# arpg/Kangaroo

Hardware: AMD Instinct MI355X
Metric: kinectfusion_frames_per_sec_640x480_to_512cubed_tsdf (higher is better)
Workload: dtype f32

## Files before the change

include/kfx_debug.h:

```cpp
#ifndef KFX_DEBUG_H
#define KFX_DEBUG_H

#include "kfx.h"

#ifdef __cplusplus
extern "C" {
#endif

int kfx_debug_rmw(const kfx_volume* vol, int variant, kfx_stream stream);

int kfx_debug_div_uniform_check(float b, unsigned long long* d_out, kfx_stream stream);

int kfx_debug_div_core_check(unsigned seed, int per_divisor, unsigned long long* d_out, kfx_stream stream);
int kfx_debug_sqrt_core_check(unsigned long long* d_out, kfx_stream stream);
int kfx_debug_wave_xor_check(unsigned seed, unsigned long long* d_out, kfx_stream stream);

int kfx_debug_summary_export(kfx_sdf_summary* s, float tol, float vref, int fine_shift, void* R_out, void* C_out, int dims_out[12],
                             kfx_stream stream);

int kfx_debug_summary_conditional_builds(kfx_sdf_summary* s, int out[2], kfx_stream stream);

#ifdef __cplusplus
}
#endif
#endif
```

kangaroo_amd/csrc/debug.hip:

```cpp
#include "kfx_device.h"
#include "sampling.h"
#include "../../include/kfx_debug.h"

namespace kfx {

__global__ __launch_bounds__(256) void k_rmw_linear(float4* __restrict__ base, size_t n4)
{
    const size_t stride = (size_t)gridDim.x * blockDim.x;
    for (size_t i = (size_t)blockIdx.x * blockDim.x + threadIdx.x; i < n4; i += stride) {
        float4 c = base[i];
        c.y += 1.0f;
        c.w += 1.0f;
        base[i] = c;
    }
}

template <int ZC>
__global__ __launch_bounds__(256) void k_rmw_brick(unsigned char* vptr, size_t pitch, size_t img_pitch, int X, int Y, int Z)
{
    const int tid = threadIdx.x, lane = tid & 63, wv = tid >> 6;
    const int x0 = (blockIdx.x * 32 + (lane & 31)) * 2;
    const int y = blockIdx.y * 8 + wv * 2 + (lane >> 5);
    const int zbeg = blockIdx.z * ZC, zend = min(zbeg + ZC, Z);
    if (x0 >= X || y >= Y) return;
// ... 203 lines not shown
    }
    case 1: hipLaunchKernelGGL(k_rmw_brick<16>, dim3(ceil_div(X, 64), ceil_div(Y, 8), ceil_div(Z, 16)), dim3(256), 0, s, p, vol->pitch, vol->img_pitch, X, Y, Z); break;
    case 2: hipLaunchKernelGGL(k_rmw_rows<16>, dim3(ceil_div(X, 128), ceil_div(Y, 4), ceil_div(Z, 16)), dim3(256), 0, s, p, vol->pitch, vol->img_pitch, X, Y, Z); break;
    case 3: hipLaunchKernelGGL(k_rmw_column, dim3(ceil_div(X, 128), ceil_div(Y, 4), 1), dim3(256), 0, s, p, vol->pitch, vol->img_pitch, X, Y, Z); break;
    case 4: hipLaunchKernelGGL(k_rmw_brick<64>, dim3(ceil_div(X, 64), ceil_div(Y, 8), ceil_div(Z, 64)), dim3(256), 0, s, p, vol->pitch, vol->img_pitch, X, Y, Z); break;
    case 5: hipLaunchKernelGGL(k_rmw_rows<4>, dim3(ceil_div(X, 128), ceil_div(Y, 4), ceil_div(Z, 4)), dim3(256), 0, s, p, vol->pitch, vol->img_pitch, X, Y, Z); break;
#define GEN(ID, WX, WY, ZC, NT) \
    case ID: hipLaunchKernelGGL((k_rmw_gen<WX, WY, ZC, NT>), dim3(ceil_div(X, 128 * WX), ceil_div(Y, WY), ceil_div(Z, ZC)), dim3(256), 0, s, p, vol->pitch, vol->img_pitch, X, Y, Z); break;
    GEN(10, 4, 1, 16, false)
    GEN(11, 2, 2, 16, false)
    GEN(12, 1, 4, 16, false)
    GEN(13, 1, 4, 16, true)
    GEN(14, 4, 1, 16, true)
    GEN(15, 1, 4, 1, false)
    GEN(16, 1, 4, 64, false)
    GEN(17, 4, 1, 4, false)
    GEN(18, 2, 2, 16, true)
#undef GEN
    default: return set_error(KFX_E_RANGE, "kfx_debug_rmw: variant");
    }
    return check_launch("kfx_debug_rmw");
}

extern "C" int kfx_debug_summary_export(kfx_sdf_summary* s, float tol, float vref, int fine_shift, void* R_out, void* C_out, int dims_out[12],
                                        kfx_stream stream)
{
    if (!s || !dims_out) return set_error(KFX_E_NULL, "kfx_debug_summary_export: null argument");
    if (fine_shift < 3 || fine_shift > 5) return set_error(KFX_E_RANGE, "kfx_debug_summary_export: fine_shift in [3, 5]");
    ClassView cv;
    summary_class_layout(s, fine_shift, cv);
    dims_out[0] = s->nbx; dims_out[1] = s->nby; dims_out[2] = s->nbz;
    dims_out[3] = cv.fine.first; dims_out[4] = cv.fine.rw; dims_out[5] = cv.fine.ny;
    dims_out[6] = cv.coarse.first; dims_out[7] = cv.coarse.rw; dims_out[8] = cv.coarse.ny;
    dims_out[9] = cv.words; dims_out[10] = s->n_coarse; dims_out[11] = (s->h_skippable && s->builds) ? ((volatile int*)s->h_skippable)[(s->builds - 1) % KFX_SUMMARY_RING] : -2;
    const size_t n = (size_t)s->nbx * s->nby * s->nbz;
    hipStream_t st = (hipStream_t)stream;
    if (R_out && hipMemcpyAsync(R_out, s->R, n * sizeof(float4), hipMemcpyDeviceToDevice, st) != hipSuccess) return set_error(KFX_E_RANGE, "kfx_debug_summary_export: copy");
    if (C_out) {
        if (int e = summary_classes_prepare(s, tol, vref, fine_shift, st)) return e;
        if (hipMemcpyAsync(C_out, s->C, (size_t)cv.words * sizeof(unsigned), hipMemcpyDeviceToDevice, st) != hipSuccess || hipStreamSynchronize(st) != hipSuccess)
            return set_error(KFX_E_RANGE, "kfx_debug_summary_export: copy");
        dims_out[11] = (s->h_skippable && s->builds) ? ((volatile int*)s->h_skippable)[(s->builds - 1) % KFX_SUMMARY_RING] : -2;
    }
    return 0;
}

extern "C" int kfx_debug_summary_conditional_builds(kfx_sdf_summary* s, int out[2], kfx_stream stream)
{
    if (!s || !out) return set_error(KFX_E_NULL, "kfx_debug_summary_conditional_builds: null argument");
    hipStream_t st = (hipStream_t)stream;
    if (hipMemcpyAsync(out, s->d_count + 3, 2 * sizeof(int), hipMemcpyDeviceToHost, st) != hipSuccess || hipStreamSynchronize(st) != hipSuccess)
        return set_error(KFX_E_RANGE, "kfx_debug_summary_conditional_builds: copy");
    return 0;
}
```

kangaroo_amd/csrc/kfx_device.h:

```cpp
#pragma once

#include <hip/hip_runtime.h>
#include <stddef.h>
#include <stdint.h>

#include "../../include/kfx.h"
#include "../../include/kfx_extras.h"
#include "../../include/kfx_summary_h.h"

namespace kfx {

struct V3 { float x, y, z; };

__device__ __forceinline__ V3 v3(float x, float y, float z) { return V3{x, y, z}; }
__device__ __forceinline__ V3 operator+(V3 a, V3 b) { return V3{a.x + b.x, a.y + b.y, a.z + b.z}; }
__device__ __forceinline__ V3 operator-(V3 a, V3 b) { return V3{a.x - b.x, a.y - b.y, a.z - b.z}; }
__device__ __forceinline__ V3 operator*(V3 a, float s) { return V3{a.x * s, a.y * s, a.z * s}; }
__device__ __forceinline__ V3 div_cw(V3 a, V3 b) { return V3{a.x / b.x, a.y / b.y, a.z / b.z}; }
__device__ __forceinline__ V3 div_s(V3 a, float s) { const float inv = 1.0f / s; return a * inv; }
__device__ __forceinline__ float dot(V3 a, V3 b) { return a.x * b.x + a.y * b.y + a.z * b.z; }
__device__ __forceinline__ float length(V3 a) { return sqrtf(dot(a, a)); }
__device__ __forceinline__ float lerp(float a, float b, float t) { return a + t * (b - a); }
__device__ __forceinline__ V3 lerp(V3 a, V3 b, float t) { return a + (b - a) * t; }
__device__ __forceinline__ float clampf(float f, float a, float b) { return fmaxf(a, fminf(f, b)); }
// ... 138 lines not shown
};

__host__ __device__ inline int ceil_div(int a, int b) { return (a + b - 1) / b; }

}

#define KFX_SUMMARY_RING 8
struct kfx_sdf_summary {
    float4* R;
    int nbx, nby, nbz;
    int w, h, d;
    int cell_bytes;
    const unsigned char* base;
    size_t pitch, img_pitch;
    unsigned* C;
    int c_dirty;
    float c_lo_ok, c_hi_ok;
    float c_tol, c_vref;
    int c_shift;
    int c_global;
    int n_coarse;
    int* d_count;
    int* d_dirty;
    int* h_skippable;
    int* d_skippable;
    hipEvent_t build_done[8];
    unsigned builds;
    unsigned plain_calls;
    unsigned sweeps;
};
namespace kfx {
struct ClassLevel {
    int shift;
    int ny;
    int rw;
    int first;
};
struct ClassView {
    const unsigned* C;
    ClassLevel fine, coarse;
    int words;
    float vref;
    float tol;
    int amb_ok;
    int ox, oy, oz;
    float eps;
    int nx5, nz5, top_n, lds_words;
    int global, top_first;
};
__device__ __forceinline__ unsigned brick_class_mask(const float lo, const float hi, const int state, const float lo_ok, const float hi_ok)
{
    const bool in_band = lo >= lo_ok && hi <= hi_ok;
    return (state == 1 ? 1u : 0u) | ((state == 0 && in_band) ? 2u : 0u) | ((state == 1 || in_band) ? 4u : 0u);
}
inline __host__ __device__ void class_level_up(const int nx, const int ny, const int nz, const int shift, const int first, ClassLevel& L, int& ux, int& uz, int& words)
{
    ux = (nx + 1) >> 1; uz = (nz + 1) >> 1;
    L.shift = shift; L.ny = (ny + 1) >> 1; L.rw = 2 * ((ux + 31) >> 5); L.first = first;
    words = (L.rw * L.ny * uz + 3) & ~3;
}
__device__ __forceinline__ void classes_level_up(unsigned* tab, const ClassLevel& src, int snx, int snz, const ClassLevel& dst, int dnx, int dnz)
{
    const int lane = threadIdx.x & 63;
    int lg = 0;
    while ((1 << lg) < dnx && lg < 6) ++lg;
    const int chunks = (dnx + 63) >> 6;
    const int px = chunks > 1 ? chunks << 6 : 1 << lg;
    const int total = px * dst.ny * dnz;
    for (int e0 = 0; e0 < total; e0 += 256) {
        const int e = e0 + (int)threadIdx.x;
        const int bx = chunks > 1 ? e % px : e & (px - 1), r = chunks > 1 ? e / px : e >> lg;
        const int by = r % dst.ny, bz = r / dst.ny;
        int cls = 0;
        if (e < total && bx < dnx) {
            bool all_free = true, all_nan = true, all_either = true;
#pragma unroll
            for (int k = 0; k < 8; ++k) {
                const int x = min(2 * bx + (k & 1), snx - 1), y = min(2 * by + ((k >> 1) & 1), src.ny - 1), z = min(2 * bz + (k >> 2), snz - 1);
                const uint2 w = *reinterpret_cast<const uint2*>(tab + src.first + (z * src.ny + y) * src.rw + ((x >> 5) << 1));
                const int c = (int)((w.x >> (x & 31)) & 1u) | (int)(((w.y >> (x & 31)) & 1u) << 1);
                all_free = all_free && c == 1;
                all_nan = all_nan && c == 2;
                all_either = all_either && c != 0;
            }
            cls = all_free ? 1 : (all_nan ? 2 : (all_either ? 3 : 0));
        }
        const unsigned long long p0 = __ballot(cls & 1), p1 = __ballot(cls & 2);
        if (e < total && (bx & 63) == 0 && (chunks > 1 || bx == 0)) {
            const int sh = chunks > 1 ? 0 : lane;
            const unsigned long long m = (chunks > 1 || lg == 6) ? ~0ull : ((1ull << (1 << lg)) - 1ull);
            const unsigned long long r0 = (p0 >> sh) & m, r1 = (p1 >> sh) & m;
            unsigned* out = tab + dst.first + (bz * dst.ny + by) * dst.rw + (bx >> 6) * 4;
            out[0] = (unsigned)r0; out[1] = (unsigned)r1;
            if ((bx >> 6) * 4 + 2 < dst.rw) { out[2] = (unsigned)(r0 >> 32); out[3] = (unsigned)(r1 >> 32); }
        }
    }
}
int summary_classes_prepare(kfx_sdf_summary* s, float tol, float vref, int fine_shift, hipStream_t stream, int global = 0);
void summary_class_layout(const kfx_sdf_summary* s, int fine_shift, ClassView& cv);
void summary_top_layout(const ClassView& cv, ClassLevel& l6, ClassLevel& l7, int& w6, int& w7);
int summary_view_offset(const kfx_sdf_summary* s, const kfx_volume* view, int* ox, int* oy, int* oz);
}

namespace kfx {
int set_error(int code, const char* what);
int check_launch(const char* what);
int math_mode();
size_t texel_image_bytes(size_t w, size_t h);
int depth_to_vbo_normals_texels(const kfx_image* vbo, const kfx_image* nrm, const kfx_image* depth, const float K[4], float scale,
                                const kfx_image* texels, kfx_stream stream);
int sdf_fuse_slab_texels(const kfx_volume* vol, const kfx_slab* slab, const kfx_image* depth, const kfx_image* norm, const kfx_image* texels,
                         const float T_cw[12], const float K[4], float trunc_dist, float max_w, float mincostheta, unsigned flags, kfx_stream stream);
int sdf_fuse_texels(const kfx_volume* vol, kfx_sdf_summary* summary, const kfx_image* depth, const kfx_image* norm, const kfx_image* texels,
                    const float T_cw[12], const float K[4], float trunc_dist, float max_w, float mincostheta, unsigned flags, kfx_stream stream);
}
```

kangaroo_amd/csrc/raycast.hip:

```cpp
#include <cmath>

#include <hip/hip_fp16.h>

#include "kfx_device.h"
#include "sampling.h"

namespace kfx {

struct RayParams {
    VolView vol;
    V3 size;
    V3 dims1;
    V3 hi2;
    V3 voxel;
    V3 inv_size;
    int fastdiv, off32;
    Pose T;
    Intr K;
    unsigned char *dptr, *nptr, *iptr;
    size_t dpitch, npitch, ipitch;
    int w, h;
    float near, far, trunc;
    int subpix;
    int tile_log2w;
// ... 659 lines not shown
    if (int e = check_volume(vol, CELL::BYTES, 3, VOLUME_MAX_DIM, "RaycastSdf")) return e;
    set_geometry(p, vol);
    set_voxel_size(p, vol);
    for (int i = 0; i < 12; ++i) p.T.m[i] = T_wc[i];
    p.K = Intr{K[0], K[1], K[2], K[3]};
    p.dptr = (unsigned char*)depth->ptr;
    p.nptr = (unsigned char*)norm->ptr;
    p.iptr = (unsigned char*)img->ptr;
    p.dpitch = depth->pitch;
    p.npitch = norm->pitch;
    p.ipitch = img->pitch;
    p.w = (int)img->w;
    p.h = (int)img->h;
    p.near = near;
    p.far = far;
    p.trunc = trunc_dist;
    p.subpix = subpix ? 1 : 0;
    p.tile_log2w = 5;
    p.wg_log2x = 1;
    p.sparse_lanes = 0;
    return 0;
}

template <typename CELL>
static int class_view(ClassView& cl, size_t* lds_bytes, int* usable, kfx_sdf_summary* summary, const kfx_volume* vol, const RayParams& p, kfx_stream stream,
                      bool allow_global = true)
{
    *usable = 0;
    if (int e = summary_view_offset(summary, vol, &cl.ox, &cl.oy, &cl.oz)) return e;
    if (!(p.trunc > 0.f) || !(p.trunc < __builtin_inff())) return 0;
    static const int kb_env = env_int("KFX_RAYCAST_CLASS_KB", 16, 1, 60);
    static const int gt_env = env_int("KFX_RAYCAST_GLOBAL_TABLES", 0);
    static const int top_env = env_int("KFX_RAYCAST_TOP_LEVELS", 2, 0, 2);
    int fine = 3;
    for (; fine < 5; ++fine) {
        summary_class_layout(summary, fine, cl);
        if ((size_t)cl.words * 4 <= (size_t)kb_env * 1024) break;
    }
    auto top_levels = [&](int& w6, int& w7) {
        summary_class_layout(summary, fine, cl);
        cl.nx5 = ceil_div(summary->w, 32); cl.nz5 = ceil_div(summary->d, 32);
        ClassLevel l6, l7;
        summary_top_layout(cl, l6, l7, w6, w7);
        const int nx6 = (cl.nx5 + 1) >> 1, nz6 = (cl.nz5 + 1) >> 1;
        cl.top_n = 0;
        if (cl.nx5 > 1 || cl.coarse.ny > 1 || cl.nz5 > 1) cl.top_n = 1;
// ... 5 lines not shown
    const size_t lds_static = sizeof(RayParams) + sizeof(TopLevels) + 2048;
    const int derived = (cl.top_n > 0 ? w6 : 0) + (cl.top_n > 1 ? w7 : 0);
    cl.global = gt_env > 0 || (size_t)cl.words * 4 > 60 * 1024 || (size_t)(cl.words + derived) * 4 + lds_static > 64 * 1024;
    if (cl.global) {
        fine = 4;
        top_levels(w6, w7);
        cl.top_first = cl.words;
        cl.lds_words = (cl.top_n > 0 ? w6 : 0) + (cl.top_n > 1 ? w7 : 0);
        if ((size_t)cl.lds_words * 4 + lds_static > 64 * 1024) return 0;
    } else {
        cl.top_first = 0;
        cl.lds_words = cl.words + derived;
    }
    if (cl.global && !allow_global) return 0;
    const bool half = CELL::BYTES == 4;
    const float vref = half ? __half2float(__float2half_rn(p.trunc)) : p.trunc;
    const float tol = math_mode() == KFX_MATH_FAST ? (half ? KFX_SUMMARY_HALF_BAND : 1e-5f) : 0.f;
    static const int force_env = env_int("KFX_RAYCAST_SUMMARY", 0);
    if (force_env < 0) return 0;
    const bool steer = force_env == 0 && summary->h_skippable;
    if (steer && summary->plain_calls && (summary->plain_calls++ % 8u) != 0u) return 0;
    if (int e = summary_classes_prepare(summary, tol, vref, fine, (hipStream_t)stream, cl.global)) return e;
    if (steer && summary->builds >= 3) {
        const unsigned ref = (summary->builds - 3) % KFX_SUMMARY_RING;
        (void)hipEventSynchronize(summary->build_done[ref]);
        const int known = ((volatile int*)summary->h_skippable)[ref];
        if (known >= 0 && (long long)known * 4 < summary->n_coarse) {
            if (!summary->plain_calls) summary->plain_calls = 1;
            return 0;
        }
        summary->plain_calls = 0;
    }
    cl.C = summary->C;
    cl.vref = vref;
    cl.amb_ok = fmaxf(vref, p.voxel.x) == p.trunc ? 1 : 0;
    cl.tol = tol;
    const double u24 = 1.0 / 16777216.0;
    double eps = 0.0;
    const float bmin[3] = {p.vol.bmin.x, p.vol.bmin.y, p.vol.bmin.z}, bmax[3] = {p.vol.bmax.x, p.vol.bmax.y, p.vol.bmax.z};
    const float size[3] = {p.size.x, p.size.y, p.size.z}, dims1[3] = {p.dims1.x, p.dims1.y, p.dims1.z};
    const float cw[3] = {p.T.m[3], p.T.m[7], p.T.m[11]};
    for (int a = 0; a < 3; ++a) {
        if (!(size[a] > 0.f)) return 0;
        const double sc = (double)dims1[a] / size[a];
        const double pmax = std::fmax(std::fabs((double)bmin[a]), std::fabs((double)bmax[a])), ca = std::fabs((double)cw[a]);
        const double A = std::fabs(((double)cw[a] - bmin[a]) * sc);
        const double t = sc * (3.0 * pmax + 2.0 * ca + size[a]) * u24 + 2.0 * dims1[a] * u24;
        const double e = u24 * (3.0 * A + 2.0 * sc * (pmax + ca) + dims1[a]) + 3.0 * u24 * (dims1[a] + A);
        eps = std::fmax(eps, t + e);
// ... 347 lines not shown
```

kangaroo_amd/csrc/summary.hip:

```cpp
#include <algorithm>
#include <new>

#include <hip/hip_fp16.h>

#include "kfx_device.h"

namespace kfx {

__global__ __launch_bounds__(256) void k_summary_fill(float4* __restrict__ R, size_t n, float lo, float hi, int state)
{
    const size_t i = (size_t)blockIdx.x * 256 + threadIdx.x;
    if (i < n) R[i] = make_float4(lo, hi, __int_as_float(state), 0.f);
}

struct ClassBuild {
    const float4* R;
    unsigned* C;
    int nbx, nby, nbz;
    int shift, nx, ny, nz, rw;
    float lo_ok, hi_ok;
    const unsigned* src;
    int src_shift, src_nx, src_ny, src_nz, src_rw;
};
struct TopBuild {
    int on;
    unsigned* tab;
    ClassLevel l5, l6, l7;
    int nx5, nz5, nx6, nz6, nx7, nz7;
};
template <int M>
__device__ __forceinline__ int class_row(const ClassBuild& b, const long long wave)
{
    const float4* __restrict__ R = b.R;
    unsigned* __restrict__ C = b.C;
    const unsigned* __restrict__ src = b.src;
    const int nbx = b.nbx, nby = b.nby, nbz = b.nbz, shift = b.shift, nx = b.nx, ny = b.ny, rw = b.rw;
    const int src_shift = b.src_shift, src_nx = b.src_nx, src_ny = b.src_ny, src_nz = b.src_nz, src_rw = b.src_rw;
    const float lo_ok = b.lo_ok, hi_ok = b.hi_ok;
    const int lane = threadIdx.x & 63;
    const int chunks = (nx + 63) >> 6;
    const int chunk = (int)(wave % chunks), by = (int)((wave / chunks) % ny), bz = (int)(wave / ((long long)chunks * ny));
    const int bx = chunk * 64 + lane;
    int cls = 0;
    if (bx < nx) {
        bool all_nan = true, all_free = true, all_either = true;
        if constexpr (M == 0) {
            const int m = 1 << (shift - src_shift);
            for (int z0 = 0; z0 < m; z0 += 2) {
                uint2 w2[2][4];
#pragma unroll
                for (int dz = 0; dz < 2; ++dz)
// ... 34 lines not shown
                    for (int dx = 0; dx <= M; ++dx)
                        r[(dz * (M + 1) + dy) * (M + 1) + dx] =
                            R[((size_t)min(bz * M + dz, nbz - 1) * nby + min(by * M + dy, nby - 1)) * nbx + min(bx * M + dx, nbx - 1)];
#pragma unroll
            for (int k = 0; k < (M + 1) * (M + 1) * (M + 1); ++k) {
                const unsigned m = brick_class_mask(r[k].x, r[k].y, __float_as_int(r[k].z), lo_ok, hi_ok);
                all_nan = all_nan && (m & 1u);
                all_free = all_free && (m & 2u);
                all_either = all_either && (m & 4u);
            }
        }
        cls = all_free ? 1 : (all_nan ? 2 : (all_either ? 3 : 0));
    }
    const unsigned long long p0 = __ballot(cls & 1), p1 = __ballot(cls & 2);
    if (lane == 0) {
        unsigned* row = C + ((size_t)bz * ny + by) * rw + chunk * 4;
        row[0] = (unsigned)p0; row[1] = (unsigned)p1;
        if (chunk * 4 + 2 < rw) { row[2] = (unsigned)(p0 >> 32); row[3] = (unsigned)(p1 >> 32); }
    }
    return __popcll(p0 | p1);
}

template <int M>
__global__ __launch_bounds__(256) void k_summary_classes(const ClassBuild b, const long long n_waves, const int* __restrict__ dirty)
{
    if (dirty && *dirty == 0) return;
    const long long wave = (long long)blockIdx.x * 4 + (threadIdx.x >> 6);
    if (wave < n_waves) class_row<M>(b, wave);
}

template <int M>
__global__ __launch_bounds__(256) void k_summary_classes_coarse(const ClassBuild b, const long long n_waves, int* __restrict__ count, int* __restrict__ publish,
                                                                int* __restrict__ dirty, const int conditional, const TopBuild t)
{
    __shared__ int s_count[4];
    __shared__ int s_last;
    if (conditional && *dirty == 0) {
        if (blockIdx.x == 0 && threadIdx.x == 0) {
            __hip_atomic_store(publish, count[2], __ATOMIC_RELAXED, __HIP_MEMORY_SCOPE_SYSTEM);
            count[4] += 1;
        }
        return;
    }
    const int wv = threadIdx.x >> 6;
    const long long wave = (long long)blockIdx.x * 4 + wv;
    const int n = wave < n_waves ? class_row<M>(b, wave) : 0;
    if ((threadIdx.x & 63) == 0) s_count[wv] = n;
    __threadfence();
    __syncthreads();
    if (threadIdx.x == 0) {
        s_last = 0;
        atomicAdd(&count[0], s_count[0] + s_count[1] + s_count[2] + s_count[3]);
        __threadfence();
        if (atomicAdd(&count[1], 1) == (int)gridDim.x - 1) {
            __threadfence();
            s_last = 1;
            const int total = atomicExch(&count[0], 0);
            count[1] = 0;
            count[2] = total;
            if (conditional) count[3] += 1;
            *dirty = 0;
            __hip_atomic_store(publish, total, __ATOMIC_RELAXED, __HIP_MEMORY_SCOPE_SYSTEM);
        }
    }
    __syncthreads();
    if (t.on && s_last) {
        __threadfence();
        classes_level_up(t.tab, t.l5, t.nx5, t.nz5, t.l6, t.nx6, t.nz6);
        __threadfence();
        __syncthreads();
        classes_level_up(t.tab, t.l6, t.nx6, t.nz6, t.l7, t.nx7, t.nz7);
    }
}

template <int BYTES>
__global__ __launch_bounds__(256) void k_summary_rebuild(float4* __restrict__ R, const unsigned char* __restrict__ base, size_t pitch, size_t img_pitch,
                                                         int w, int h, int d, int nbx, int nby, int nbz, int aligned16)
{
    const long long brick = (long long)blockIdx.x * 4 + (threadIdx.x >> 6);
    if (brick >= (long long)nbx * nby * nbz) return;
    const int lane = threadIdx.x & 63;
    const int bx = (int)(brick % nbx), by = (int)((brick / nbx) % nby), bz = (int)(brick / ((long long)nbx * nby));
    const int y = by * 8 + (lane & 7), z = bz * 8 + (lane >> 3), x0 = bx * 8;
    float lo = __builtin_inff(), hi = -__builtin_inff();
    bool nan = false, val = false;
    if (y < h && z < d) {
        const unsigned char* row = base + (size_t)z * img_pitch + (size_t)y * pitch + (size_t)x0 * BYTES;
        if (BYTES == 4 && x0 + 8 <= w && aligned16) {
            uint4 c[2];
#pragma unroll
            for (int k = 0; k < 2; ++k) c[k] = reinterpret_cast<const uint4*>(row)[k];
#pragma unroll
            for (int k = 0; k < 2; ++k) {
                const unsigned u[4] = {c[k].x, c[k].y, c[k].z, c[k].w};
// ... 51 lines not shown
}
static int class_level_words(const ClassLevel& L, int d) { return L.rw * L.ny * ceil_div(d, 1 << L.shift); }

void summary_class_layout(const kfx_sdf_summary* s, int fine_shift, ClassView& cv)
{
    class_level(cv.fine, fine_shift, s->w, s->h, 0);
    const int fw = fine_shift < 5 ? class_level_words(cv.fine, s->d) : 0;
    class_level(cv.coarse, 5, s->w, s->h, (fw + 3) & ~3);
    cv.words = cv.coarse.first + ((class_level_words(cv.coarse, s->d) + 3) & ~3);
}

void summary_top_layout(const ClassView& cv, ClassLevel& l6, ClassLevel& l7, int& w6, int& w7)
{
    int nx6, nz6, nx7, nz7;
    class_level_up(cv.nx5, cv.coarse.ny, cv.nz5, 6, cv.words, l6, nx6, nz6, w6);
    class_level_up(nx6, l6.ny, nz6, 7, cv.words + w6, l7, nx7, nz7, w7);
}

int summary_classes_prepare(kfx_sdf_summary* s, float tol, float vref, int fine_shift, hipStream_t stream, int global)
{
    const bool same = s->c_tol == tol && s->c_vref == vref && s->c_shift == fine_shift && s->c_global == global;
    if (!s->c_dirty && same) return 0;
    const int conditional = (s->c_dirty == 1 && same && !global) ? 1 : 0;
    const int* fine_dirty = conditional ? s->d_dirty : nullptr;
    ClassView cv;
    summary_class_layout(s, fine_shift, cv);
    cv.nx5 = ceil_div(s->w, 32); cv.nz5 = ceil_div(s->d, 32);
    ClassLevel l6, l7;
    int w6, w7;
    summary_top_layout(cv, l6, l7, w6, w7);
    TopBuild top{};
    top.on = global ? 0 : 1;
    top.tab = s->C;
    top.l5 = cv.coarse; top.l6 = l6; top.l7 = l7;
    top.nx5 = cv.nx5; top.nz5 = cv.nz5;
    top.nx6 = (top.nx5 + 1) >> 1; top.nz6 = (top.nz5 + 1) >> 1;
    top.nx7 = (top.nx6 + 1) >> 1; top.nz7 = (top.nz6 + 1) >> 1;
    const float lo_ok = vref - tol * vref, hi_ok = vref + tol * vref;
    for (int pass = 0; pass < (global ? 4 : 2); ++pass) {
        if (pass >= 2) {
            const ClassLevel& L = pass == 2 ? l6 : l7;
            const ClassLevel& S = pass == 2 ? cv.coarse : l6;
            ClassBuild b;
            b.R = s->R; b.C = s->C + L.first;
            b.nbx = s->nbx; b.nby = s->nby; b.nbz = s->nbz;
            b.shift = L.shift; b.nx = ceil_div(s->w, 1 << L.shift); b.ny = L.ny; b.nz = ceil_div(s->d, 1 << L.shift); b.rw = L.rw;
            b.lo_ok = lo_ok; b.hi_ok = hi_ok;
            b.src = s->C + S.first;
            b.src_shift = S.shift; b.src_nx = ceil_div(s->w, 1 << S.shift); b.src_ny = S.ny; b.src_nz = ceil_div(s->d, 1 << S.shift); b.src_rw = S.rw;
            const long long waves = (long long)ceil_div(b.nx, 64) * b.ny * b.nz;
            hipLaunchKernelGGL(k_summary_classes<0>, dim3((unsigned)((waves + 3) / 4)), dim3(256), 0, stream, b, waves, (const int*)nullptr);
            if (int e = check_launch("kfx_sdf_summary (classes)")) return e;
            continue;
        }
        const ClassLevel& L = pass ? cv.coarse : cv.fine;
        if (!pass && fine_shift >= 5) continue;
        ClassBuild b;
        b.R = s->R; b.C = s->C + L.first;
        b.nbx = s->nbx; b.nby = s->nby; b.nbz = s->nbz;
        b.shift = L.shift; b.nx = ceil_div(s->w, 1 << L.shift); b.ny = L.ny; b.nz = ceil_div(s->d, 1 << L.shift); b.rw = L.rw;
        b.lo_ok = lo_ok; b.hi_ok = hi_ok;
        const bool from_fine = pass && fine_shift < 5;
        b.src = from_fine ? s->C + cv.fine.first : nullptr;
        b.src_shift = cv.fine.shift; b.src_nx = ceil_div(s->w, 1 << cv.fine.shift); b.src_ny = cv.fine.ny;
        b.src_nz = ceil_div(s->d, 1 << cv.fine.shift); b.src_rw = cv.fine.rw;
        const long long waves = (long long)ceil_div(b.nx, 64) * b.ny * b.nz;
        if (pass) {
            const dim3 grid((unsigned)((waves + 3) / 4));
            const unsigned slot = s->builds % KFX_SUMMARY_RING;
            int* publish = s->d_skippable + (s->h_skippable ? slot : 0);
            if (from_fine) hipLaunchKernelGGL(k_summary_classes_coarse<0>, grid, dim3(256), 0, stream, b, waves, s->d_count, publish, s->d_dirty, conditional, top);
            else hipLaunchKernelGGL(k_summary_classes_coarse<4>, grid, dim3(256), 0, stream, b, waves, s->d_count, publish, s->d_dirty, conditional, top);
            if (s->h_skippable) (void)hipEventRecord(s->build_done[slot], stream);
            s->builds += 1;
        } else if (L.shift == 3) {
            hipLaunchKernelGGL(k_summary_classes<1>, dim3((unsigned)((waves + 3) / 4)), dim3(256), 0, stream, b, waves, fine_dirty);
        } else {
            hipLaunchKernelGGL(k_summary_classes<2>, dim3((unsigned)((waves + 3) / 4)), dim3(256), 0, stream, b, waves, fine_dirty);
        }
        if (int e = check_launch("kfx_sdf_summary (classes)")) return e;
    }
    s->c_dirty = 0; s->c_tol = tol; s->c_vref = vref; s->c_shift = fine_shift; s->c_global = global;
    s->c_lo_ok = lo_ok; s->c_hi_ok = hi_ok;
    return 0;
}

int summary_view_offset(const kfx_sdf_summary* s, const kfx_volume* view, int* ox, int* oy, int* oz)
{
    if (!s || !view || !view->ptr) return set_error(KFX_E_NULL, "summary: null argument");
    if (view->pitch != s->pitch || view->img_pitch != s->img_pitch) return set_error(KFX_E_SHAPE, "summary: the volume is not a view of the summary's volume (pitches)");
    const unsigned char* q = static_cast<const unsigned char*>(view->ptr);
    if (q < s->base) return set_error(KFX_E_SHAPE, "summary: the volume is not a view of the summary's volume");
    const size_t off = (size_t)(q - s->base);
    const size_t z = off / s->img_pitch, rem = off % s->img_pitch, y = rem / s->pitch, xb = rem % s->pitch;
    const size_t cb = (size_t)s->cell_bytes;
    if (xb % cb || z + view->d > (size_t)s->d || y + view->h > (size_t)s->h || xb / cb + view->w > (size_t)s->w)
        return set_error(KFX_E_SHAPE, "summary: the volume is not a view of the summary's volume (extent)");
    *ox = (int)(xb / cb); *oy = (int)y; *oz = (int)z;
    return 0;
}

}

using namespace kfx;

static int summary_create(kfx_sdf_summary** out, const kfx_volume* vol, int cell_bytes)
{
    if (!out || !vol || !vol->ptr) return set_error(KFX_E_NULL, "kfx_sdf_summary_create: null argument");
    if (vol->w < 2 || vol->h < 2 || vol->d < 2 || vol->w > 65535 || vol->h > 65535 || vol->d > 65535) return set_error(KFX_E_SHAPE, "kfx_sdf_summary_create: volume dimensions");
    kfx_sdf_summary* s = new (std::nothrow) kfx_sdf_summary;
    if (!s) return set_error(KFX_E_RANGE, "kfx_sdf_summary_create: out of memory");
    s->nbx = ceil_div((int)vol->w, 8); s->nby = ceil_div((int)vol->h, 8); s->nbz = ceil_div((int)vol->d, 8);
    s->w = (int)vol->w; s->h = (int)vol->h; s->d = (int)vol->d;
    s->cell_bytes = cell_bytes;
    s->base = static_cast<const unsigned char*>(vol->ptr);
    s->pitch = vol->pitch; s->img_pitch = vol->img_pitch;
    s->R = nullptr; s->C = nullptr; s->d_count = nullptr; s->h_skippable = nullptr; s->d_skippable = nullptr;
    s->c_dirty = 2; s->c_tol = -1.f; s->c_vref = 0.f; s->c_shift = 0; s->c_global = 0; s->sweeps = 0;
    s->c_lo_ok = 0.f; s->c_hi_ok = 0.f; s->d_dirty = nullptr;
    s->builds = 0; s->plain_calls = 0;
    for (auto& e : s->build_done) e = nullptr;
    s->n_coarse = ceil_div(s->w, 32) * ceil_div(s->h, 32) * ceil_div(s->d, 32);
    const size_t n = (size_t)s->nbx * s->nby * s->nbz;
    ClassView cv;
    summary_class_layout(s, 3, cv);
    cv.nx5 = ceil_div(s->w, 32); cv.nz5 = ceil_div(s->d, 32);
    ClassLevel l6, l7;
    int w6, w7;
    summary_top_layout(cv, l6, l7, w6, w7);
    const int words = cv.words + w6 + w7;
    bool ok = hipMalloc((void**)&s->R, n * sizeof(float4)) == hipSuccess && hipMalloc((void**)&s->C, (size_t)words * sizeof(unsigned)) == hipSuccess &&
              hipMalloc((void**)&s->d_count, 64 * sizeof(int)) == hipSuccess && hipMemset(s->d_count, 0, 64 * sizeof(int)) == hipSuccess;
    if (ok) s->d_dirty = s->d_count + 32;
    if (ok && hipHostMalloc((void**)&s->h_skippable, KFX_SUMMARY_RING * sizeof(int), hipHostMallocMapped) == hipSuccess) {
        for (int i = 0; i < KFX_SUMMARY_RING; ++i) s->h_skippable[i] = -1;
        bool evs = hipHostGetDevicePointer((void**)&s->d_skippable, s->h_skippable, 0) == hipSuccess;
        for (int i = 0; evs && i < KFX_SUMMARY_RING; ++i) evs = hipEventCreateWithFlags(&s->build_done[i], hipEventDisableTiming) == hipSuccess;
        if (!evs) {
            for (auto& e : s->build_done) { if (e) (void)hipEventDestroy(e); e = nullptr; }
            (void)hipHostFree(s->h_skippable);
            s->h_skippable = nullptr;
        }
    } else {
        s->h_skippable = nullptr;
    }
    if (ok && !s->h_skippable) {
        (void)hipGetLastError();
        ok = hipMalloc((void**)&s->d_skippable, sizeof(int)) == hipSuccess;
    }
    if (!ok) {
        (void)hipGetLastError();
        kfx_sdf_summary_destroy(s);
        return set_error(KFX_E_NODEVICE, "kfx_sdf_summary_create: hipMalloc");
    }
    *out = s;
    return kfx_sdf_summary_invalidate(s, nullptr);
}

extern "C" int kfx_sdf_summary_create(kfx_sdf_summary** out, const kfx_volume* vol) { return summary_create(out, vol, 8); }
extern "C" int kfx_sdf_summary_create_h(kfx_sdf_summary** out, const kfx_volume* vol) { return summary_create(out, vol, 4); }

extern "C" int kfx_sdf_summary_destroy(kfx_sdf_summary* s)
{
    if (!s) return 0;
    (void)hipDeviceSynchronize();
    if (s->R) (void)hipFree(s->R);
    if (s->C) (void)hipFree(s->C);
    if (s->d_count) (void)hipFree(s->d_count);
    for (auto& e : s->build_done) if (e) (void)hipEventDestroy(e);
    if (s->h_skippable) (void)hipHostFree(s->h_skippable);
    else if (s->d_skippable) (void)hipFree(s->d_skippable);
    delete s;
    return 0;
}

extern "C" int kfx_sdf_summary_rebuild(kfx_sdf_summary* s, kfx_stream stream)
{
    if (!s) return set_error(KFX_E_NULL, "kfx_sdf_summary_rebuild: null summary");
    const long long n = (long long)s->nbx * s->nby * s->nbz;
    const int aligned16 = ((((uintptr_t)s->base) | s->pitch | s->img_pitch) & 15) == 0;
    if (s->cell_bytes == 4)
        hipLaunchKernelGGL(k_summary_rebuild<4>, dim3((unsigned)((n + 3) / 4)), dim3(256), 0, (hipStream_t)stream, s->R, s->base, s->pitch, s->img_pitch,
                           s->w, s->h, s->d, s->nbx, s->nby, s->nbz, aligned16);
    else
        hipLaunchKernelGGL(k_summary_rebuild<8>, dim3((unsigned)((n + 3) / 4)), dim3(256), 0, (hipStream_t)stream, s->R, s->base, s->pitch, s->img_pitch,
                           s->w, s->h, s->d, s->nbx, s->nby, s->nbz, aligned16);
    s->c_dirty = 2;
    return check_launch("kfx_sdf_summary_rebuild");
}

extern "C" int kfx_sdf_summary_invalidate(kfx_sdf_summary* s, kfx_stream stream)
{
// ... 35 lines not shown
```

Measured before the change: 2475.

## Fuse class-table build levels into one kernel and publish tagged counts

The fine and coarse class-table passes (and the top levels) are merged into a single kernel. The last block to finish builds the coarse level from the fine one, then combines the higher levels. The per-build hipEvent record and hipEventSynchronize are replaced by a tagged 64-bit count in coherent mapped host memory, which the host polls, falling back to hipStreamQuery. This cuts kernel launches and event overhead per frame, at the cost of a serial last-block tail and busy-wait polling on the host.

```diff
diff --git a/include/kfx_debug.h b/include/kfx_debug.h
--- a/include/kfx_debug.h
+++ b/include/kfx_debug.h
@@ -20,6 +20,10 @@
 
 int kfx_debug_summary_conditional_builds(kfx_sdf_summary* s, int out[2], kfx_stream stream);
 
+int kfx_debug_summary_export_levels(kfx_sdf_summary* s, float tol, float vref, int fine_shift, void* C_out, int dims_out[28], kfx_stream stream);
+
+int kfx_debug_summary_build_ops(const kfx_sdf_summary* s, unsigned long long out[2]);
+
 #ifdef __cplusplus
 }
 #endif
diff --git a/kangaroo_amd/csrc/debug.hip b/kangaroo_amd/csrc/debug.hip
--- a/kangaroo_amd/csrc/debug.hip
+++ b/kangaroo_amd/csrc/debug.hip
@@ -249,6 +249,12 @@
     return check_launch("kfx_debug_rmw");
 }
 
+static int last_published_count(const kfx_sdf_summary* s)
+{
+    if (!s->h_skippable || !s->builds) return -2;
+    return (int)(unsigned)__atomic_load_n(s->h_skippable + (s->builds - 1) % KFX_SUMMARY_RING, __ATOMIC_ACQUIRE);
+}
+
 extern "C" int kfx_debug_summary_export(kfx_sdf_summary* s, float tol, float vref, int fine_shift, void* R_out, void* C_out, int dims_out[12],
                                         kfx_stream stream)
 {
@@ -259,7 +265,7 @@
     dims_out[0] = s->nbx; dims_out[1] = s->nby; dims_out[2] = s->nbz;
     dims_out[3] = cv.fine.first; dims_out[4] = cv.fine.rw; dims_out[5] = cv.fine.ny;
     dims_out[6] = cv.coarse.first; dims_out[7] = cv.coarse.rw; dims_out[8] = cv.coarse.ny;
-    dims_out[9] = cv.words; dims_out[10] = s->n_coarse; dims_out[11] = (s->h_skippable && s->builds) ? ((volatile int*)s->h_skippable)[(s->builds - 1) % KFX_SUMMARY_RING] : -2;
+    dims_out[9] = cv.words; dims_out[10] = s->n_coarse; dims_out[11] = last_published_count(s);
     const size_t n = (size_t)s->nbx * s->nby * s->nbz;
     hipStream_t st = (hipStream_t)stream;
     if (R_out && hipMemcpyAsync(R_out, s->R, n * sizeof(float4), hipMemcpyDeviceToDevice, st) != hipSuccess) return set_error(KFX_E_RANGE, "kfx_debug_summary_export: copy");
@@ -267,7 +273,7 @@
         if (int e = summary_classes_prepare(s, tol, vref, fine_shift, st)) return e;
         if (hipMemcpyAsync(C_out, s->C, (size_t)cv.words * sizeof(unsigned), hipMemcpyDeviceToDevice, st) != hipSuccess || hipStreamSynchronize(st) != hipSuccess)
             return set_error(KFX_E_RANGE, "kfx_debug_summary_export: copy");
-        dims_out[11] = (s->h_skippable && s->builds) ? ((volatile int*)s->h_skippable)[(s->builds - 1) % KFX_SUMMARY_RING] : -2;
+        dims_out[11] = last_published_count(s);
     }
     return 0;
 }
@@ -280,3 +286,41 @@
         return set_error(KFX_E_RANGE, "kfx_debug_summary_conditional_builds: copy");
     return 0;
 }
+
+extern "C" int kfx_debug_summary_export_levels(kfx_sdf_summary* s, float tol, float vref, int fine_shift, void* C_out, int dims_out[28], kfx_stream stream)
+{
+    if (!s || !dims_out) return set_error(KFX_E_NULL, "kfx_debug_summary_export_levels: null argument");
+    if (fine_shift < 3 || fine_shift > 5) return set_error(KFX_E_RANGE, "kfx_debug_summary_export_levels: fine_shift in [3, 5]");
+    ClassView cv;
+    summary_class_layout(s, fine_shift, cv);
+    cv.nx5 = ceil_div(s->w, 32); cv.nz5 = ceil_div(s->d, 32);
+    ClassLevel l6, l7;
+    int w6, w7;
+    summary_top_layout(cv, l6, l7, w6, w7);
+    const int nx6 = (cv.nx5 + 1) >> 1, nz6 = (cv.nz5 + 1) >> 1;
+    const ClassLevel* lv[4] = {&cv.fine, &cv.coarse, &l6, &l7};
+    const int nx[4] = {ceil_div(s->w, 1 << cv.fine.shift), cv.nx5, nx6, (nx6 + 1) >> 1};
+    const int nz[4] = {ceil_div(s->d, 1 << cv.fine.shift), cv.nz5, nz6, (nz6 + 1) >> 1};
+    int n = 0;
+    for (int k = fine_shift < 5 ? 0 : 1; k < 4; ++k, ++n) {
+        int* d = dims_out + 4 + 6 * n;
+        d[0] = lv[k]->shift; d[1] = lv[k]->first; d[2] = lv[k]->rw; d[3] = lv[k]->ny; d[4] = nx[k]; d[5] = nz[k];
+    }
+    const int words = cv.words + w6 + w7;
+    dims_out[0] = n; dims_out[1] = words; dims_out[2] = last_published_count(s); dims_out[3] = s->n_coarse;
+    if (C_out) {
+        hipStream_t st = (hipStream_t)stream;
+        if (int e = summary_classes_prepare(s, tol, vref, fine_shift, st)) return e;
+        if (hipMemcpyAsync(C_out, s->C, (size_t)words * sizeof(unsigned), hipMemcpyDeviceToDevice, st) != hipSuccess || hipStreamSynchronize(st) != hipSuccess)
+            return set_error(KFX_E_RANGE, "kfx_debug_summary_export_levels: copy");
+        dims_out[2] = last_published_count(s);
+    }
+    return 0;
+}
+
+extern "C" int kfx_debug_summary_build_ops(const kfx_sdf_summary* s, unsigned long long out[2])
+{
+    if (!s || !out) return set_error(KFX_E_NULL, "kfx_debug_summary_build_ops: null argument");
+    out[0] = s->build_launches; out[1] = s->build_events;
+    return 0;
+}
diff --git a/kangaroo_amd/csrc/kfx_device.h b/kangaroo_amd/csrc/kfx_device.h
--- a/kangaroo_amd/csrc/kfx_device.h
+++ b/kangaroo_amd/csrc/kfx_device.h
@@ -184,13 +184,15 @@
     int n_coarse;
     int* d_count;
     int* d_dirty;
-    int* h_skippable;
-    int* d_skippable;
-    hipEvent_t build_done[8];
+    unsigned long long* h_skippable;
+    unsigned long long* d_skippable;
+    hipStream_t build_stream[KFX_SUMMARY_RING];
     unsigned builds;
     unsigned plain_calls;
     unsigned sweeps;
-};
+    unsigned long long build_launches, build_events;
+};
+inline __host__ __device__ unsigned long long kfx_ring_pair(int count, unsigned tag) { return ((unsigned long long)tag << 32) | (unsigned)count; }
 namespace kfx {
 struct ClassLevel {
     int shift;
@@ -221,43 +223,6 @@
     L.shift = shift; L.ny = (ny + 1) >> 1; L.rw = 2 * ((ux + 31) >> 5); L.first = first;
     words = (L.rw * L.ny * uz + 3) & ~3;
 }
-__device__ __forceinline__ void classes_level_up(unsigned* tab, const ClassLevel& src, int snx, int snz, const ClassLevel& dst, int dnx, int dnz)
-{
-    const int lane = threadIdx.x & 63;
-    int lg = 0;
-    while ((1 << lg) < dnx && lg < 6) ++lg;
-    const int chunks = (dnx + 63) >> 6;
-    const int px = chunks > 1 ? chunks << 6 : 1 << lg;
-    const int total = px * dst.ny * dnz;
-    for (int e0 = 0; e0 < total; e0 += 256) {
-        const int e = e0 + (int)threadIdx.x;
-        const int bx = chunks > 1 ? e % px : e & (px - 1), r = chunks > 1 ? e / px : e >> lg;
-        const int by = r % dst.ny, bz = r / dst.ny;
-        int cls = 0;
-        if (e < total && bx < dnx) {
-            bool all_free = true, all_nan = true, all_either = true;
-#pragma unroll
-            for (int k = 0; k < 8; ++k) {
-                const int x = min(2 * bx + (k & 1), snx - 1), y = min(2 * by + ((k >> 1) & 1), src.ny - 1), z = min(2 * bz + (k >> 2), snz - 1);
-                const uint2 w = *reinterpret_cast<const uint2*>(tab + src.first + (z * src.ny + y) * src.rw + ((x >> 5) << 1));
-                const int c = (int)((w.x >> (x & 31)) & 1u) | (int)(((w.y >> (x & 31)) & 1u) << 1);
-                all_free = all_free && c == 1;
-                all_nan = all_nan && c == 2;
-                all_either = all_either && c != 0;
-            }
-            cls = all_free ? 1 : (all_nan ? 2 : (all_either ? 3 : 0));
-        }
-        const unsigned long long p0 = __ballot(cls & 1), p1 = __ballot(cls & 2);
-        if (e < total && (bx & 63) == 0 && (chunks > 1 || bx == 0)) {
-            const int sh = chunks > 1 ? 0 : lane;
-            const unsigned long long m = (chunks > 1 || lg == 6) ? ~0ull : ((1ull << (1 << lg)) - 1ull);
-            const unsigned long long r0 = (p0 >> sh) & m, r1 = (p1 >> sh) & m;
-            unsigned* out = tab + dst.first + (bz * dst.ny + by) * dst.rw + (bx >> 6) * 4;
-            out[0] = (unsigned)r0; out[1] = (unsigned)r1;
-            if ((bx >> 6) * 4 + 2 < dst.rw) { out[2] = (unsigned)(r0 >> 32); out[3] = (unsigned)(r1 >> 32); }
-        }
-    }
-}
 int summary_classes_prepare(kfx_sdf_summary* s, float tol, float vref, int fine_shift, hipStream_t stream, int global = 0);
 void summary_class_layout(const kfx_sdf_summary* s, int fine_shift, ClassView& cv);
 void summary_top_layout(const ClassView& cv, ClassLevel& l6, ClassLevel& l7, int& w6, int& w7);
diff --git a/kangaroo_amd/csrc/raycast.hip b/kangaroo_amd/csrc/raycast.hip
--- a/kangaroo_amd/csrc/raycast.hip
+++ b/kangaroo_amd/csrc/raycast.hip
@@ -705,6 +705,31 @@
     return 0;
 }
 
+static int published_count(const kfx_sdf_summary* s, unsigned build, int* count)
+{
+    const unsigned long long* slot = s->h_skippable + build % KFX_SUMMARY_RING;
+    const auto read = [&] {
+        const unsigned long long v = __atomic_load_n(slot, __ATOMIC_ACQUIRE);
+        *count = (int)(unsigned)v;
+        return (unsigned)(v >> 32) == build + 1u;
+    };
+    for (;;) {
+        for (int k = 0; k < 256; ++k)
+            if (read()) return 0;
+        const hipError_t q = hipStreamQuery(s->build_stream[build % KFX_SUMMARY_RING]);
+        if (q == hipErrorNotReady) {
+            (void)hipGetLastError();
+            continue;
+        }
+        if (q != hipSuccess) {
+            (void)hipGetLastError();
+            return set_error((int)q, "RaycastSdf(tracked): the stream of a class-table build");
+        }
+        if (read()) return 0;
+        return set_error(KFX_E_RANGE, "RaycastSdf(tracked): a finished class-table build has not published its count");
+    }
+}
+
 template <typename CELL>
 static int class_view(ClassView& cl, size_t* lds_bytes, int* usable, kfx_sdf_summary* summary, const kfx_volume* vol, const RayParams& p, kfx_stream stream,
                       bool allow_global = true)
@@ -756,9 +781,8 @@
     if (steer && summary->plain_calls && (summary->plain_calls++ % 8u) != 0u) return 0;
     if (int e = summary_classes_prepare(summary, tol, vref, fine, (hipStream_t)stream, cl.global)) return e;
     if (steer && summary->builds >= 3) {
-        const unsigned ref = (summary->builds - 3) % KFX_SUMMARY_RING;
-        (void)hipEventSynchronize(summary->build_done[ref]);
-        const int known = ((volatile int*)summary->h_skippable)[ref];
+        int known;
+        if (int e = published_count(summary, summary->builds - 3, &known)) return e;
         if (known >= 0 && (long long)known * 4 < summary->n_coarse) {
             if (!summary->plain_calls) summary->plain_calls = 1;
             return 0;
diff --git a/kangaroo_amd/csrc/summary.hip b/kangaroo_amd/csrc/summary.hip
--- a/kangaroo_amd/csrc/summary.hip
+++ b/kangaroo_amd/csrc/summary.hip
@@ -25,8 +25,8 @@
 struct TopBuild {
     int on;
     unsigned* tab;
-    ClassLevel l5, l6, l7;
-    int nx5, nz5, nx6, nz6, nx7, nz7;
+    ClassLevel lf, l5, l6, l7;
+    int nxf, nzf, nx5, nz5, nx6, nz6, nx7, nz7;
 };
 template <int M>
 __device__ __forceinline__ int class_row(const ClassBuild& b, const long long wave)
@@ -107,22 +107,133 @@
 }
 
 template <int M>
-__global__ __launch_bounds__(256) void k_summary_classes(const ClassBuild b, const long long n_waves, const int* __restrict__ dirty)
-{
-    if (dirty && *dirty == 0) return;
+__global__ __launch_bounds__(256) void k_summary_classes(const ClassBuild b, const long long n_waves)
+{
     const long long wave = (long long)blockIdx.x * 4 + (threadIdx.x >> 6);
     if (wave < n_waves) class_row<M>(b, wave);
 }
 
 template <int M>
-__global__ __launch_bounds__(256) void k_summary_classes_coarse(const ClassBuild b, const long long n_waves, int* __restrict__ count, int* __restrict__ publish,
-                                                                int* __restrict__ dirty, const int conditional, const TopBuild t)
+__device__ __forceinline__ int classes_combine(unsigned* tab, const ClassLevel& src, int snx, int snz, const ClassLevel& dst, int dnx, int dnz)
+{
+    const int lane = threadIdx.x & 63;
+    int lg = 0;
+    while ((1 << lg) < dnx && lg < 6) ++lg;
+    const int chunks = (dnx + 63) >> 6;
+    const int px = chunks > 1 ? chunks << 6 : 1 << lg;
+    const int total = px * dst.ny * dnz;
+    int n = 0;
+    for (int e0 = 0; e0 < total; e0 += 256) {
+        const int e = e0 + (int)threadIdx.x;
+        const int bx = chunks > 1 ? e % px : e & (px - 1), r = chunks > 1 ? e / px : e >> lg;
+        const int by = r % dst.ny, bz = r / dst.ny;
+        int cls = 0;
+        if (e < total && bx < dnx) {
+            bool all_free = true, all_nan = true, all_either = true;
+            uint2 w[M][M];
+#pragma unroll
+            for (int dz = 0; dz < M; ++dz)
+#pragma unroll
+                for (int dy = 0; dy < M; ++dy) {
+                    const int z = min(M * bz + dz, snz - 1), y = min(M * by + dy, src.ny - 1);
+                    w[dz][dy] = *reinterpret_cast<const uint2*>(tab + src.first + (z * src.ny + y) * src.rw + (((bx * M) >> 5) << 1));
+                }
+#pragma unroll
+            for (int dz = 0; dz < M; ++dz)
+#pragma unroll
+                for (int dy = 0; dy < M; ++dy)
+#pragma unroll
+                    for (int dx = 0; dx < M; ++dx) {
+                        const int x = min(bx * M + dx, snx - 1);
+                        const int c = (int)((w[dz][dy].x >> (x & 31)) & 1u) | (int)(((w[dz][dy].y >> (x & 31)) & 1u) << 1);
+                        all_free = all_free && c == 1;
+                        all_nan = all_nan && c == 2;
+                        all_either = all_either && c != 0;
+                    }
+            cls = all_free ? 1 : (all_nan ? 2 : (all_either ? 3 : 0));
+        }
+        const unsigned long long p0 = __ballot(cls & 1), p1 = __ballot(cls & 2);
+        if (e < total && (bx & 63) == 0 && (chunks > 1 || bx == 0)) {
+            const int sh = chunks > 1 ? 0 : lane;
+            const unsigned long long m = (chunks > 1 || lg == 6) ? ~0ull : ((1ull << (1 << lg)) - 1ull);
+            const unsigned long long r0 = (p0 >> sh) & m, r1 = (p1 >> sh) & m;
+            unsigned* out = tab + dst.first + (bz * dst.ny + by) * dst.rw + (bx >> 6) * 4;
+            out[0] = (unsigned)r0; out[1] = (unsigned)r1;
+            if ((bx >> 6) * 4 + 2 < dst.rw) { out[2] = (unsigned)(r0 >> 32); out[3] = (unsigned)(r1 >> 32); }
+            n += __popcll(r0 | r1);
+        }
+    }
+    return n;
+}
+
+__device__ __forceinline__ void classes_top_levels(const TopBuild& t)
+{
+    classes_combine<2>(t.tab, t.l5, t.nx5, t.nz5, t.l6, t.nx6, t.nz6);
+    __threadfence();
+    __syncthreads();
+    classes_combine<2>(t.tab, t.l6, t.nx6, t.nz6, t.l7, t.nx7, t.nz7);
+}
+
+template <int M, int M5>
+__global__ __launch_bounds__(256) void k_summary_classes_all(const ClassBuild b, const long long n_waves, int* __restrict__ count,
+                                                             unsigned long long* __restrict__ publish, const unsigned tag, int* __restrict__ dirty,
+                                                             const int conditional, const TopBuild t)
+{
+    __shared__ int s_last, s_total;
+    if (conditional && *dirty == 0) {
+        if (blockIdx.x == 0 && threadIdx.x == 0) {
+            __hip_atomic_store(publish, kfx_ring_pair(count[2], tag), __ATOMIC_RELAXED, __HIP_MEMORY_SCOPE_SYSTEM);
+            count[4] += 1;
+        }
+        return;
+    }
+    const long long wave = (long long)blockIdx.x * 4 + (threadIdx.x >> 6);
+    if (wave < n_waves) class_row<M>(b, wave);
+    __threadfence();
+    asm volatile("s_waitcnt vmcnt(0)" ::: "memory");
+    __syncthreads();
+    if (threadIdx.x == 0) {
+        s_total = 0;
+        s_last = atomicAdd(&count[1], 1) == (int)gridDim.x - 1 ? 1 : 0;
+    }
+    __syncthreads();
+    if (!s_last) return;
+    __threadfence();
+    {
+        unsigned* fine = t.tab + t.lf.first;
+        const int words = t.lf.rw * t.lf.ny * t.nzf;
+        unsigned any = 0;
+        for (int i = (int)threadIdx.x * 4; i < words; i += 1024) {
+            const uint4 v = *reinterpret_cast<const uint4*>(fine + i);
+            any |= v.x | v.y | v.z | v.w;
+        }
+        asm volatile("" ::"v"(any));
+    }
+    const int n = classes_combine<M5>(t.tab, t.lf, t.nxf, t.nzf, t.l5, t.nx5, t.nz5);
+    if (n) atomicAdd(&s_total, n);
+    __threadfence();
+    __syncthreads();
+    if (threadIdx.x == 0) {
+        const int total = s_total;
+        count[1] = 0;
+        count[2] = total;
+        if (conditional) count[3] += 1;
+        *dirty = 0;
+        __hip_atomic_store(publish, kfx_ring_pair(total, tag), __ATOMIC_RELAXED, __HIP_MEMORY_SCOPE_SYSTEM);
+    }
+    classes_top_levels(t);
+}
+
+template <int M>
+__global__ __launch_bounds__(256) void k_summary_classes_coarse(const ClassBuild b, const long long n_waves, int* __restrict__ count,
+                                                                unsigned long long* __restrict__ publish, const unsigned tag, int* __restrict__ dirty,
+                                                                const int conditional, const TopBuild t)
 {
     __shared__ int s_count[4];
     __shared__ int s_last;
     if (conditional && *dirty == 0) {
         if (blockIdx.x == 0 && threadIdx.x == 0) {
-            __hip_atomic_store(publish, count[2], __ATOMIC_RELAXED, __HIP_MEMORY_SCOPE_SYSTEM);
+            __hip_atomic_store(publish, kfx_ring_pair(count[2], tag), __ATOMIC_RELAXED, __HIP_MEMORY_SCOPE_SYSTEM);
             count[4] += 1;
         }
         return;
@@ -145,16 +256,13 @@
             count[2] = total;
             if (conditional) count[3] += 1;
             *dirty = 0;
-            __hip_atomic_store(publish, total, __ATOMIC_RELAXED, __HIP_MEMORY_SCOPE_SYSTEM);
+            __hip_atomic_store(publish, kfx_ring_pair(total, tag), __ATOMIC_RELAXED, __HIP_MEMORY_SCOPE_SYSTEM);
         }
     }
     __syncthreads();
     if (t.on && s_last) {
         __threadfence();
-        classes_level_up(t.tab, t.l5, t.nx5, t.nz5, t.l6, t.nx6, t.nz6);
-        __threadfence();
-        __syncthreads();
-        classes_level_up(t.tab, t.l6, t.nx6, t.nz6, t.l7, t.nx7, t.nz7);
+        classes_top_levels(t);
     }
 }
 
@@ -252,7 +360,6 @@
     const bool same = s->c_tol == tol && s->c_vref == vref && s->c_shift == fine_shift && s->c_global == global;
     if (!s->c_dirty && same) return 0;
     const int conditional = (s->c_dirty == 1 && same && !global) ? 1 : 0;
-    const int* fine_dirty = conditional ? s->d_dirty : nullptr;
     ClassView cv;
     summary_class_layout(s, fine_shift, cv);
     cv.nx5 = ceil_div(s->w, 32); cv.nz5 = ceil_div(s->d, 32);
@@ -262,53 +369,62 @@
     TopBuild top{};
     top.on = global ? 0 : 1;
     top.tab = s->C;
-    top.l5 = cv.coarse; top.l6 = l6; top.l7 = l7;
+    top.lf = cv.fine; top.l5 = cv.coarse; top.l6 = l6; top.l7 = l7;
+    top.nxf = ceil_div(s->w, 1 << cv.fine.shift); top.nzf = ceil_div(s->d, 1 << cv.fine.shift);
     top.nx5 = cv.nx5; top.nz5 = cv.nz5;
     top.nx6 = (top.nx5 + 1) >> 1; top.nz6 = (top.nz5 + 1) >> 1;
     top.nx7 = (top.nx6 + 1) >> 1; top.nz7 = (top.nz6 + 1) >> 1;
     const float lo_ok = vref - tol * vref, hi_ok = vref + tol * vref;
-    for (int pass = 0; pass < (global ? 4 : 2); ++pass) {
-        if (pass >= 2) {
-            const ClassLevel& L = pass == 2 ? l6 : l7;
-            const ClassLevel& S = pass == 2 ? cv.coarse : l6;
-            ClassBuild b;
-            b.R = s->R; b.C = s->C + L.first;
-            b.nbx = s->nbx; b.nby = s->nby; b.nbz = s->nbz;
-            b.shift = L.shift; b.nx = ceil_div(s->w, 1 << L.shift); b.ny = L.ny; b.nz = ceil_div(s->d, 1 << L.shift); b.rw = L.rw;
-            b.lo_ok = lo_ok; b.hi_ok = hi_ok;
-            b.src = s->C + S.first;
-            b.src_shift = S.shift; b.src_nx = ceil_div(s->w, 1 << S.shift); b.src_ny = S.ny; b.src_nz = ceil_div(s->d, 1 << S.shift); b.src_rw = S.rw;
-            const long long waves = (long long)ceil_div(b.nx, 64) * b.ny * b.nz;
-            hipLaunchKernelGGL(k_summary_classes<0>, dim3((unsigned)((waves + 3) / 4)), dim3(256), 0, stream, b, waves, (const int*)nullptr);
-            if (int e = check_launch("kfx_sdf_summary (classes)")) return e;
-            continue;
-        }
-        const ClassLevel& L = pass ? cv.coarse : cv.fine;
-        if (!pass && fine_shift >= 5) continue;
-        ClassBuild b;
+    const auto build_of = [&](const ClassLevel& L, const ClassLevel* S) {
+        ClassBuild b{};
         b.R = s->R; b.C = s->C + L.first;
         b.nbx = s->nbx; b.nby = s->nby; b.nbz = s->nbz;
         b.shift = L.shift; b.nx = ceil_div(s->w, 1 << L.shift); b.ny = L.ny; b.nz = ceil_div(s->d, 1 << L.shift); b.rw = L.rw;
         b.lo_ok = lo_ok; b.hi_ok = hi_ok;
-        const bool from_fine = pass && fine_shift < 5;
-        b.src = from_fine ? s->C + cv.fine.first : nullptr;
-        b.src_shift = cv.fine.shift; b.src_nx = ceil_div(s->w, 1 << cv.fine.shift); b.src_ny = cv.fine.ny;
-        b.src_nz = ceil_div(s->d, 1 << cv.fine.shift); b.src_rw = cv.fine.rw;
-        const long long waves = (long long)ceil_div(b.nx, 64) * b.ny * b.nz;
-        if (pass) {
-            const dim3 grid((unsigned)((waves + 3) / 4));
-            const unsigned slot = s->builds % KFX_SUMMARY_RING;
-            int* publish = s->d_skippable + (s->h_skippable ? slot : 0);
-            if (from_fine) hipLaunchKernelGGL(k_summary_classes_coarse<0>, grid, dim3(256), 0, stream, b, waves, s->d_count, publish, s->d_dirty, conditional, top);
-            else hipLaunchKernelGGL(k_summary_classes_coarse<4>, grid, dim3(256), 0, stream, b, waves, s->d_count, publish, s->d_dirty, conditional, top);
-            if (s->h_skippable) (void)hipEventRecord(s->build_done[slot], stream);
-            s->builds += 1;
-        } else if (L.shift == 3) {
-            hipLaunchKernelGGL(k_summary_classes<1>, dim3((unsigned)((waves + 3) / 4)), dim3(256), 0, stream, b, waves, fine_dirty);
-        } else {
-            hipLaunchKernelGGL(k_summary_classes<2>, dim3((unsigned)((waves + 3) / 4)), dim3(256), 0, stream, b, waves, fine_dirty);
-        }
+        if (S) {
+            b.src = s->C + S->first;
+            b.src_shift = S->shift; b.src_nx = ceil_div(s->w, 1 << S->shift); b.src_ny = S->ny; b.src_nz = ceil_div(s->d, 1 << S->shift); b.src_rw = S->rw;
+        }
+        return b;
+    };
+    const auto waves_of = [](const ClassBuild& b) { return (long long)ceil_div(b.nx, 64) * b.ny * b.nz; };
+    const auto grid_of = [](long long waves) { return dim3((unsigned)((waves + 3) / 4)); };
+    const unsigned slot = s->builds % KFX_SUMMARY_RING, tag = s->builds + 1;
+    unsigned long long* publish = s->d_skippable + (s->h_skippable ? slot : 0);
+    s->build_stream[slot] = stream;
+    s->builds += 1;
+    if (!global && fine_shift < 5) {
+        const ClassBuild b = build_of(cv.fine, nullptr);
+        const long long waves = waves_of(b);
+        if (fine_shift == 3) hipLaunchKernelGGL((k_summary_classes_all<1, 4>), grid_of(waves), dim3(256), 0, stream, b, waves, s->d_count, publish, tag, s->d_dirty, conditional, top);
+        else hipLaunchKernelGGL((k_summary_classes_all<2, 2>), grid_of(waves), dim3(256), 0, stream, b, waves, s->d_count, publish, tag, s->d_dirty, conditional, top);
+        s->build_launches += 1;
         if (int e = check_launch("kfx_sdf_summary (classes)")) return e;
+    } else {
+        const bool from_fine = fine_shift < 5;
+        if (from_fine) {
+            const ClassBuild b = build_of(cv.fine, nullptr);
+            const long long waves = waves_of(b);
+            if (fine_shift == 3) hipLaunchKernelGGL(k_summary_classes<1>, grid_of(waves), dim3(256), 0, stream, b, waves);
+            else hipLaunchKernelGGL(k_summary_classes<2>, grid_of(waves), dim3(256), 0, stream, b, waves);
+            s->build_launches += 1;
+            if (int e = check_launch("kfx_sdf_summary (classes)")) return e;
+        }
+        {
+            const ClassBuild b = build_of(cv.coarse, from_fine ? &cv.fine : nullptr);
+            const long long waves = waves_of(b);
+            if (from_fine) hipLaunchKernelGGL(k_summary_classes_coarse<0>, grid_of(waves), dim3(256), 0, stream, b, waves, s->d_count, publish, tag, s->d_dirty, conditional, top);
+            else hipLaunchKernelGGL(k_summary_classes_coarse<4>, grid_of(waves), dim3(256), 0, stream, b, waves, s->d_count, publish, tag, s->d_dirty, conditional, top);
+            s->build_launches += 1;
+            if (int e = check_launch("kfx_sdf_summary (classes)")) return e;
+        }
+        for (int k = 0; global && k < 2; ++k) {
+            const ClassBuild b = build_of(k ? l7 : l6, k ? &l6 : &cv.coarse);
+            const long long waves = waves_of(b);
+            hipLaunchKernelGGL(k_summary_classes<0>, grid_of(waves), dim3(256), 0, stream, b, waves);
+            s->build_launches += 1;
+            if (int e = check_launch("kfx_sdf_summary (classes)")) return e;
+        }
     }
     s->c_dirty = 0; s->c_tol = tol; s->c_vref = vref; s->c_shift = fine_shift; s->c_global = global;
     s->c_lo_ok = lo_ok; s->c_hi_ok = hi_ok;
@@ -349,7 +465,8 @@
     s->c_dirty = 2; s->c_tol = -1.f; s->c_vref = 0.f; s->c_shift = 0; s->c_global = 0; s->sweeps = 0;
     s->c_lo_ok = 0.f; s->c_hi_ok = 0.f; s->d_dirty = nullptr;
     s->builds = 0; s->plain_calls = 0;
-    for (auto& e : s->build_done) e = nullptr;
+    s->build_launches = 0; s->build_events = 0;
+    for (auto& q : s->build_stream) q = nullptr;
     s->n_coarse = ceil_div(s->w, 32) * ceil_div(s->h, 32) * ceil_div(s->d, 32);
     const size_t n = (size_t)s->nbx * s->nby * s->nbz;
     ClassView cv;
@@ -362,12 +479,9 @@
     bool ok = hipMalloc((void**)&s->R, n * sizeof(float4)) == hipSuccess && hipMalloc((void**)&s->C, (size_t)words * sizeof(unsigned)) == hipSuccess &&
               hipMalloc((void**)&s->d_count, 64 * sizeof(int)) == hipSuccess && hipMemset(s->d_count, 0, 64 * sizeof(int)) == hipSuccess;
     if (ok) s->d_dirty = s->d_count + 32;
-    if (ok && hipHostMalloc((void**)&s->h_skippable, KFX_SUMMARY_RING * sizeof(int), hipHostMallocMapped) == hipSuccess) {
-        for (int i = 0; i < KFX_SUMMARY_RING; ++i) s->h_skippable[i] = -1;
-        bool evs = hipHostGetDevicePointer((void**)&s->d_skippable, s->h_skippable, 0) == hipSuccess;
-        for (int i = 0; evs && i < KFX_SUMMARY_RING; ++i) evs = hipEventCreateWithFlags(&s->build_done[i], hipEventDisableTiming) == hipSuccess;
-        if (!evs) {
-            for (auto& e : s->build_done) { if (e) (void)hipEventDestroy(e); e = nullptr; }
+    if (ok && hipHostMalloc((void**)&s->h_skippable, KFX_SUMMARY_RING * sizeof(unsigned long long), hipHostMallocMapped | hipHostMallocCoherent) == hipSuccess) {
+        for (int i = 0; i < KFX_SUMMARY_RING; ++i) s->h_skippable[i] = kfx_ring_pair(-1, 0u);
+        if (hipHostGetDevicePointer((void**)&s->d_skippable, s->h_skippable, 0) != hipSuccess) {
             (void)hipHostFree(s->h_skippable);
             s->h_skippable = nullptr;
         }
@@ -376,7 +490,7 @@
     }
     if (ok && !s->h_skippable) {
         (void)hipGetLastError();
-        ok = hipMalloc((void**)&s->d_skippable, sizeof(int)) == hipSuccess;
+        ok = hipMalloc((void**)&s->d_skippable, sizeof(unsigned long long)) == hipSuccess;
     }
     if (!ok) {
         (void)hipGetLastError();
@@ -397,7 +511,6 @@
     if (s->R) (void)hipFree(s->R);
     if (s->C) (void)hipFree(s->C);
     if (s->d_count) (void)hipFree(s->d_count);
-    for (auto& e : s->build_done) if (e) (void)hipEventDestroy(e);
     if (s->h_skippable) (void)hipHostFree(s->h_skippable);
     else if (s->d_skippable) (void)hipFree(s->d_skippable);
     delete s;
```

New measurement: 2493, median of 6. No clear change (+0.7%).
